# argmaxinc/WhisperKit

Hardware: NVIDIA H100
Metric: RTFx (audio-sec/s) whisper-large-v3 greedy (higher is better)
Workload: dtype bf16

## Files before the change

whisperkit_b200/csrc/decoder_ops.cu:

```cuda
#include <curand_kernel.h>
#include <math.h>

#include <stdlib.h>

#include "common.cuh"
#include <algorithm>
#include "kernels.h"

namespace wk {

static constexpr int kMaxCtx = 224;

__device__ __forceinline__ float block_sum(float v, float* scratch) {
    v = warp_sum(v);
    const int warp = threadIdx.x >> 5, lane = threadIdx.x & 31, nw = (blockDim.x + 31) >> 5;
    __syncthreads();
    if (lane == 0) scratch[warp] = v;
    __syncthreads();
    float r = (lane < nw) ? scratch[lane] : 0.f;
    r = warp_sum(r);
    return r;
}
__device__ __forceinline__ float block_max(float v, float* scratch) {
    v = warp_max(v);
    const int warp = threadIdx.x >> 5, lane = threadIdx.x & 31, nw = (blockDim.x + 31) >> 5;
    __syncthreads();
    if (lane == 0) scratch[warp] = v;
    __syncthreads();
    float r = (lane < nw) ? scratch[lane] : -INFINITY;
    r = warp_max(r);
    return r;
}

__global__ void decode_slots_init_kernel(DecodeState st, RowParams* __restrict__ rp_dev, const int32_t* __restrict__ slot_ids,
                                         const int32_t* __restrict__ prompts, const RowParams* __restrict__ rp_new, BeamState bs) {
    const int i = blockIdx.x, b = slot_ids[i];
    const RowParams R = rp_new[i];
    const int n_prompt = R.prompt_len;
    for (int t = threadIdx.x; t < kMaxCtx; t += blockDim.x) {
        st.tokens[b * kMaxCtx + t] = t < n_prompt ? prompts[i * kMaxCtx + t] : 0;
        st.logprobs[b * kMaxCtx + t] = 0.f;
    }
    if (threadIdx.x == 0) {
        rp_dev[b] = R;
        st.n_tokens[b] = n_prompt;
        st.next_token[b] = n_prompt > 0 ? prompts[i * kMaxCtx + n_prompt - 1] : 0;
        st.done[b] = 0;
        st.first_low[b] = 0;
        st.steps[b] = 0;
        st.input_ids[b] = 0;
        st.error[b] = 0;
        st.lang_token[b] = -1;
        st.lang_logprob[b] = 0.f;
        st.lang_state[b] = R.detect == 2 ? kLangLead : 0;
        st.no_speech[b] = __int_as_float(0x7fc00000);
        if (bs.beam > 1) {
            bs.sum_lp[b] = 0.f;
            if (b % bs.beam == 0) bs.n_fin[b / bs.beam] = 0;
        }
    }
}

wk_status decode_slots_init(DecodeState st, RowParams* rp_dev, const int32_t* slot_ids, const int32_t* prompts, const RowParams* rp_new,
                            int n, cudaStream_t stream, BeamState beam) {
    if (n < 1) return WK_OK;
    decode_slots_init_kernel<<<n, 64, 0, stream>>>(st, rp_dev, slot_ids, prompts, rp_new, beam);
    count_launch();
    cudaError_t e = cudaGetLastError();
    if (e != cudaSuccess) { set_error("decode_slots_init launch: %s", cudaGetErrorString(e)); return WK_ERR_CUDA; }
    return WK_OK;
}

template <typename T>
__global__ void __launch_bounds__(256)
decoder_embed_ln_kernel(const T* __restrict__ emb, const float* __restrict__ pos_emb, const float* __restrict__ gamma,
                        const float* __restrict__ beta, DecodeState st, int vocab, int ts_begin, float* __restrict__ x,
                        T* __restrict__ xn, int d, const int32_t* __restrict__ explicit_pos) {
    __shared__ float scratch[32];
    const int b = blockIdx.x, tid = threadIdx.x;
    pdl_launch_dependents();
    pdl_wait();
    int tok, pos;
    if (explicit_pos) {
        tok = st.input_ids[b];
        pos = explicit_pos[b];
    } else {
        if (st.done[b]) return;
        const int step = st.steps[b];
        const int prompt_len = st.rp[b].prompt_len;
        pos = step;
        tok = st.next_token[b];
        bool overwrite = false;
        const int lang_state = st.lang_state[b];
        if (lang_state == kLangLead) {
            tok = st.rp[b].lead_token;
        } else if (step < prompt_len) {
            const int cur = st.tokens[b * kMaxCtx + step];
            const bool is_ts = cur >= ts_begin, pred_ts = tok >= ts_begin;
            if (!(step == prompt_len - 1 && is_ts && pred_ts)) tok = cur;
            else overwrite = true;
        }
        __syncthreads();
        if (tid == 0) {
            if (overwrite) st.tokens[b * kMaxCtx + step] = tok;
            st.input_ids[b] = tok;
            if (lang_state == kLangLeadRan) st.lang_state[b] = 0;
        }
    }
    tok = min(max(tok, 0), vocab - 1);
    float v[8];
    float s = 0.f;
#pragma unroll
    for (int k = 0; k < 8; ++k) {
        const int i = tid + k * 256;
        v[k] = 0.f;
        if (i < d) {
            v[k] = T16<T>::to_f(emb[(long long)tok * d + i]) + pos_emb[(long long)pos * d + i];
            x[(long long)b * d + i] = v[k];
            s += v[k];
        }
    }
    const float mean = block_sum(s, scratch) / d;
    float q = 0.f;
#pragma unroll
    for (int k = 0; k < 8; ++k) {
        const int i = tid + k * 256;
        if (i < d) { const float a = v[k] - mean; q += a * a; }
    }
    const float rstd = rsqrtf(block_sum(q, scratch) / d + 1e-5f);
#pragma unroll
    for (int k = 0; k < 8; ++k) {
        const int i = tid + k * 256;
        if (i < d) xn[(long long)b * d + i] = T16<T>::from_f((v[k] - mean) * rstd * gamma[i] + beta[i]);
    }
}

wk_status decoder_embed_ln(const void* emb16, const float* pos, const float* gamma, const float* beta, DecodeState st, int vocab,
                           int ts_begin, float* x, void* xn, int B, int d, int dtype, const int32_t* explicit_pos, cudaStream_t stream) {
    if (d > 2048) { set_error("decoder_embed_ln: d_model %d > 2048", d); return WK_ERR_INVALID_ARGUMENT; }
    if (dtype == WK_DTYPE_F16)
        launch_k(decoder_embed_ln_kernel<__half>, dim3(B), dim3(256), 0, stream, 1, (const __half*)emb16, pos, gamma, beta, st, vocab, ts_begin, x, (__half*)xn, d, explicit_pos);
    else
        launch_k(decoder_embed_ln_kernel<__nv_bfloat16>, dim3(B), dim3(256), 0, stream, 1, (const __nv_bfloat16*)emb16, pos, gamma, beta, st, vocab, ts_begin, x, (__nv_bfloat16*)xn, d, explicit_pos);
    count_launch();
    cudaError_t e = cudaGetLastError();
    if (e != cudaSuccess) { set_error("decoder_embed_ln launch: %s", cudaGetErrorString(e)); return WK_ERR_CUDA; }
    return WK_OK;
}

static constexpr int kReduceThreads = 320;
static constexpr int kMaxSplits = 20;

template <typename T>
__global__ void __launch_bounds__(kReduceThreads)
decoder_reduce_resid_ln_kernel(const float* __restrict__ partial, int splits, int Bp, const float* __restrict__ bias,
                               const float* __restrict__ gamma, const float* __restrict__ beta, float* __restrict__ x,
                               T* __restrict__ xn, int d) {
    __shared__ float scratch[32];
    const int b = blockIdx.x, tid = threadIdx.x;
    const int d4 = d >> 2;
    pdl_launch_dependents();
    pdl_wait();
    float4 v[2];
    float s = 0.f;
#pragma unroll
    for (int k = 0; k < 2; ++k) {
        const int i4 = tid + k * kReduceThreads;
        v[k] = make_float4(0.f, 0.f, 0.f, 0.f);
        if (i4 < d4) {
            float4 p[kMaxSplits];
#pragma unroll
            for (int sp = 0; sp < kMaxSplits; ++sp)
                if (sp < splits) p[sp] = __ldcg(reinterpret_cast<const float4*>(partial + ((long long)sp * Bp + b) * d) + i4);
            float4 a = reinterpret_cast<const float4*>(x + (long long)b * d)[i4];
            if (bias) {
                const float4 bb = __ldg(reinterpret_cast<const float4*>(bias) + i4);
                a.x += bb.x; a.y += bb.y; a.z += bb.z; a.w += bb.w;
            }
#pragma unroll
            for (int sp = 0; sp < kMaxSplits; ++sp)
                if (sp < splits) { a.x += p[sp].x; a.y += p[sp].y; a.z += p[sp].z; a.w += p[sp].w; }
            v[k] = a;
            reinterpret_cast<float4*>(x + (long long)b * d)[i4] = a;
            s += a.x + a.y + a.z + a.w;
        }
    }
    const float mean = block_sum(s, scratch) / d;
    float q = 0.f;
#pragma unroll
    for (int k = 0; k < 2; ++k) {
        const int i4 = tid + k * kReduceThreads;
        if (i4 < d4) {
            const float a0 = v[k].x - mean, a1 = v[k].y - mean, a2 = v[k].z - mean, a3 = v[k].w - mean;
            q += a0 * a0 + a1 * a1 + a2 * a2 + a3 * a3;
        }
    }
    const float rstd = rsqrtf(block_sum(q, scratch) / d + 1e-5f);
#pragma unroll
    for (int k = 0; k < 2; ++k) {
        const int i4 = tid + k * kReduceThreads;
        if (i4 < d4) {
            const float4 g = __ldg(reinterpret_cast<const float4*>(gamma) + i4), bb = __ldg(reinterpret_cast<const float4*>(beta) + i4);
            uint2 pk;
            pk.x = T16<T>::pack2((v[k].x - mean) * rstd * g.x + bb.x, (v[k].y - mean) * rstd * g.y + bb.y);
            pk.y = T16<T>::pack2((v[k].z - mean) * rstd * g.z + bb.z, (v[k].w - mean) * rstd * g.w + bb.w);
            reinterpret_cast<uint2*>(xn + (long long)b * d)[i4] = pk;
        }
    }
}

wk_status decoder_reduce_resid_ln(const float* partial, int splits, int Bp, const float* bias, const float* gamma,
                                  const float* beta, float* x, void* xn, int B, int d, int dtype, cudaStream_t stream) {
    if (splits > kMaxSplits || d > 8 * kReduceThreads || (d & 3)) {
        set_error("decoder_reduce_resid_ln: unsupported splits %d / d %d", splits, d);
        return WK_ERR_INVALID_ARGUMENT;
    }
    if (dtype == WK_DTYPE_F16)
        launch_k(decoder_reduce_resid_ln_kernel<__half>, dim3(B), dim3(kReduceThreads), 0, stream, 32, partial, splits, Bp, bias, gamma, beta, x, (__half*)xn, d);
    else
        launch_k(decoder_reduce_resid_ln_kernel<__nv_bfloat16>, dim3(B), dim3(kReduceThreads), 0, stream, 32, partial, splits, Bp, bias, gamma, beta, x, (__nv_bfloat16*)xn, d);
    count_launch();
    cudaError_t e = cudaGetLastError();
    if (e != cudaSuccess) { set_error("decoder_reduce_resid_ln launch: %s", cudaGetErrorString(e)); return WK_ERR_CUDA; }
    return WK_OK;
}

template <typename T>
__global__ void __launch_bounds__(256)
decoder_reduce_bias_gelu_kernel(const float* __restrict__ partial, int splits, int Bp, const float* __restrict__ bias,
                                T* __restrict__ out, int B, int n) {
    pdl_launch_dependents();
    pdl_wait();
    const long long idx = ((long long)blockIdx.x * blockDim.x + threadIdx.x) * 4;
    if (idx >= (long long)B * n) return;
    const int b = (int)(idx / n), i = (int)(idx - (long long)b * n);
    float4 a = *reinterpret_cast<const float4*>(bias + i);
    float4 p[8];
#pragma unroll
    for (int sp = 0; sp < 8; ++sp)
        if (sp < splits) p[sp] = __ldcg(reinterpret_cast<const float4*>(partial + ((long long)sp * Bp + b) * n + i));
#pragma unroll
    for (int sp = 0; sp < 8; ++sp)
        if (sp < splits) { a.x += p[sp].x; a.y += p[sp].y; a.z += p[sp].z; a.w += p[sp].w; }
    for (int sp = 8; sp < splits; ++sp) {
        const float4 pp = __ldcg(reinterpret_cast<const float4*>(partial + ((long long)sp * Bp + b) * n + i));
        a.x += pp.x; a.y += pp.y; a.z += pp.z; a.w += pp.w;
    }
    uint2 pk;
    pk.x = T16<T>::pack2(gelu_erf(a.x), gelu_erf(a.y));
    pk.y = T16<T>::pack2(gelu_erf(a.z), gelu_erf(a.w));
    *reinterpret_cast<uint2*>(out + (long long)b * n + i) = pk;
}

wk_status decoder_reduce_bias_gelu(const float* partial, int splits, int Bp, const float* bias, void* out, int B, int n,
                                   int dtype, cudaStream_t stream) {
    const long long threads = (long long)B * n / 4;
    const unsigned grid = (unsigned)((threads + 255) / 256);
    if (dtype == WK_DTYPE_F16)
        launch_k(decoder_reduce_bias_gelu_kernel<__half>, dim3(grid), dim3(256), 0, stream, 32, partial, splits, Bp, bias, (__half*)out, B, n);
    else
        launch_k(decoder_reduce_bias_gelu_kernel<__nv_bfloat16>, dim3(grid), dim3(256), 0, stream, 32, partial, splits, Bp, bias, (__nv_bfloat16*)out, B, n);
    count_launch();
    cudaError_t e = cudaGetLastError();
    if (e != cudaSuccess) { set_error("decoder_reduce_bias_gelu launch: %s", cudaGetErrorString(e)); return WK_ERR_CUDA; }
    return WK_OK;
}

template <typename T, bool kAnc>
__global__ void __launch_bounds__(128)
decoder_self_attention_kernel(const float* __restrict__ partial, int splits, int Bp, const float* __restrict__ bq,
                              const float* __restrict__ bv, T* __restrict__ kcache, T* __restrict__ vcache,
                              const int32_t* __restrict__ pos_ptr, const int32_t* __restrict__ done,
                              T* __restrict__ out, int B, int H, int max_len, const int32_t* __restrict__ anc) {
    __shared__ float sq[64], skc[64], svc[64];
    __shared__ float sp[kMaxCtx];
    __shared__ float red[4][64];
    __shared__ float sstat[8];
    const int tid = threadIdx.x, warp = tid >> 5, lane = tid & 31;
    const int bh = blockIdx.x, b = bh / H, h = bh % H;
    pdl_launch_dependents();
    pdl_wait();
    if (done != nullptr && done[b]) return;
    const int dm = H * 64;
    const int pos = pos_ptr[b];
    const int32_t* arow = kAnc ? anc + (long long)b * max_len : nullptr;
    const long long own = (long long)bh * max_len;
    auto row_of = [&](int t) -> long long { return kAnc ? ((long long)arow[t] * H + h) * max_len + t : own + t; };
    if (warp == 0) {
        const int e = 2 * lane;
        float2 q = make_float2(bq[h * 64 + e], bq[h * 64 + e + 1]);
        float2 k = make_float2(0.f, 0.f);
        float2 v = make_float2(bv[h * 64 + e], bv[h * 64 + e + 1]);
        for (int s = 0; s < splits; ++s) {
            const float* pr = partial + ((long long)s * Bp + b) * (3LL * dm) + h * 64 + e;
            const float2 pq = *reinterpret_cast<const float2*>(pr);
            const float2 pk = *reinterpret_cast<const float2*>(pr + dm);
            const float2 pv = *reinterpret_cast<const float2*>(pr + 2 * dm);
            q.x += pq.x; q.y += pq.y; k.x += pk.x; k.y += pk.y; v.x += pv.x; v.y += pv.y;
        }
        const uint32_t k16 = T16<T>::pack2(k.x, k.y), v16 = T16<T>::pack2(v.x, v.y);
        *reinterpret_cast<uint32_t*>(kcache + (own + pos) * 64 + e) = k16;
        *reinterpret_cast<uint32_t*>(vcache + (own + pos) * 64 + e) = v16;
        const float2 kr = T16<T>::unpack2(k16), vr = T16<T>::unpack2(v16);
        sq[e] = q.x; sq[e + 1] = q.y;
        skc[e] = kr.x; skc[e + 1] = kr.y;
        svc[e] = vr.x; svc[e + 1] = vr.y;
        const float self = warp_sum(q.x * kr.x + q.y * kr.y);
        if (lane == 0) sp[pos] = self * 0.125f;
    }
    __syncthreads();
    const int sub = lane & 7, rsel = lane >> 3;
    float qv[8];
#pragma unroll
    for (int j = 0; j < 8; ++j) qv[j] = sq[sub * 8 + j];
    const T* kb = kcache + sub * 8;
#pragma unroll 4
    for (int t0 = warp * 4; t0 < pos; t0 += 16) {
        const int t = t0 + rsel;
        float acc = 0.f;
        if (t < pos) {
            const uint4 u = *reinterpret_cast<const uint4*>(kb + row_of(t) * 64);
            const float2 a0 = T16<T>::unpack2(u.x), a1 = T16<T>::unpack2(u.y), a2 = T16<T>::unpack2(u.z), a3 = T16<T>::unpack2(u.w);
            acc = qv[0] * a0.x + qv[1] * a0.y + qv[2] * a1.x + qv[3] * a1.y + qv[4] * a2.x + qv[5] * a2.y + qv[6] * a3.x + qv[7] * a3.y;
        }
        acc += __shfl_xor_sync(0xffffffffu, acc, 1);
        acc += __shfl_xor_sync(0xffffffffu, acc, 2);
        acc += __shfl_xor_sync(0xffffffffu, acc, 4);
        if (sub == 0 && t < pos) sp[t] = acc * 0.125f;
    }
    __syncthreads();
    float mx = -INFINITY;
    for (int t = tid; t <= pos; t += 128) mx = fmaxf(mx, sp[t]);
    mx = warp_max(mx);
    if (lane == 0) sstat[warp] = mx;
    __syncthreads();
    mx = fmaxf(fmaxf(sstat[0], sstat[1]), fmaxf(sstat[2], sstat[3]));
    float sm = 0.f;
    for (int t = tid; t <= pos; t += 128) {
        const float pr = __expf(sp[t] - mx);
        sp[t] = pr;
        sm += pr;
    }
    sm = warp_sum(sm);
    if (lane == 0) sstat[4 + warp] = sm;
    __syncthreads();
    const float inv = 1.f / (sstat[4] + sstat[5] + sstat[6] + sstat[7]);
    float o8[8];
#pragma unroll
    for (int j = 0; j < 8; ++j) o8[j] = 0.f;
    const T* vb = vcache + sub * 8;
#pragma unroll 4
    for (int t0 = warp * 4; t0 < pos; t0 += 16) {
        const int t = t0 + rsel;
        if (t < pos) {
            const float pr = sp[t];
            const uint4 u = *reinterpret_cast<const uint4*>(vb + row_of(t) * 64);
            const float2 a0 = T16<T>::unpack2(u.x), a1 = T16<T>::unpack2(u.y), a2 = T16<T>::unpack2(u.z), a3 = T16<T>::unpack2(u.w);
            o8[0] += pr * a0.x; o8[1] += pr * a0.y; o8[2] += pr * a1.x; o8[3] += pr * a1.y;
            o8[4] += pr * a2.x; o8[5] += pr * a2.y; o8[6] += pr * a3.x; o8[7] += pr * a3.y;
        }
    }
#pragma unroll
    for (int j = 0; j < 8; ++j) {
        o8[j] += __shfl_xor_sync(0xffffffffu, o8[j], 8);
        o8[j] += __shfl_xor_sync(0xffffffffu, o8[j], 16);
    }
    if (rsel == 0) {
#pragma unroll
        for (int j = 0; j < 8; ++j) red[warp][sub * 8 + j] = o8[j];
    }
    __syncthreads();
    if (tid < 64) {
        const float o = red[0][tid] + red[1][tid] + red[2][tid] + red[3][tid] + sp[pos] * svc[tid];
        out[(long long)b * dm + h * 64 + tid] = T16<T>::from_f(o * inv);
    }
}

wk_status decoder_self_attention(const float* partial, int splits, int Bp, const float* bq, const float* bv, void* kcache,
                                 void* vcache, const int32_t* pos, const int32_t* done, void* out, int B, int H,
                                 int max_len, int dtype, cudaStream_t stream, const int32_t* anc) {
    if (max_len > kMaxCtx) { set_error("decoder_self_attention: max_len %d > %d", max_len, kMaxCtx); return WK_ERR_INVALID_ARGUMENT; }
    const unsigned grid = (unsigned)(B * H);
    if (dtype == WK_DTYPE_F16) {
        if (anc) launch_k(decoder_self_attention_kernel<__half, true>, dim3(grid), dim3(128), 0, stream, 2, partial, splits, Bp, bq, bv, (__half*)kcache, (__half*)vcache, pos, done, (__half*)out, B, H, max_len, anc);
        else launch_k(decoder_self_attention_kernel<__half, false>, dim3(grid), dim3(128), 0, stream, 2, partial, splits, Bp, bq, bv, (__half*)kcache, (__half*)vcache, pos, done, (__half*)out, B, H, max_len, anc);
    } else {
        if (anc) launch_k(decoder_self_attention_kernel<__nv_bfloat16, true>, dim3(grid), dim3(128), 0, stream, 2, partial, splits, Bp, bq, bv, (__nv_bfloat16*)kcache, (__nv_bfloat16*)vcache, pos, done, (__nv_bfloat16*)out, B, H, max_len, anc);
        else launch_k(decoder_self_attention_kernel<__nv_bfloat16, false>, dim3(grid), dim3(128), 0, stream, 2, partial, splits, Bp, bq, bv, (__nv_bfloat16*)kcache, (__nv_bfloat16*)vcache, pos, done, (__nv_bfloat16*)out, B, H, max_len, anc);
    }
    count_launch();
    cudaError_t e = cudaGetLastError();
    if (e != cudaSuccess) { set_error("decoder_self_attention launch: %s", cudaGetErrorString(e)); return WK_ERR_CUDA; }
    return WK_OK;
}

template <bool FP8> struct CrossCfg {
    static constexpr int kRowBytes = FP8 ? 64 : 128;
    static constexpr int kRows = FP8 ? 250 : 125;
    static constexpr int kStageBytes = kRows * kRowBytes;
    static constexpr int kStages = FP8 ? 3 : 4;
    static constexpr int kLanesPerRow = kRowBytes / 16;
    static constexpr int kRowsPerWarp = 32 / kLanesPerRow;
    static constexpr int kDims = 64 / kLanesPerRow;
};
static constexpr int kCrossRows = CrossCfg<false>::kRows;
static constexpr int kCrossThreads = 160;

__device__ __forceinline__ void fp8x16_to_f32(const uint4 u, float (&x)[16]) {
    const uint32_t w[4] = {u.x, u.y, u.z, u.w};
#pragma unroll
    for (int k = 0; k < 4; ++k) {
        uint32_t lo, hi;
        fp8x4_to_half2(w[k], lo, hi);
        const float2 a = T16<__half>::unpack2(lo), b = T16<__half>::unpack2(hi);
        x[4 * k] = a.x; x[4 * k + 1] = a.y; x[4 * k + 2] = b.x; x[4 * k + 3] = b.y;
    }
}
template <typename T, bool FP8>
__device__ __forceinline__ float cross_row_dot(const uint8_t* piece, const float (&qv)[CrossCfg<FP8>::kDims]) {
    const uint4 u = *reinterpret_cast<const uint4*>(piece);
    if constexpr (FP8) {
        float x[16];
        fp8x16_to_f32(u, x);
        float acc = 0.f;
#pragma unroll
        for (int j = 0; j < 16; ++j) acc = fmaf(qv[j], x[j], acc);
        return acc;
    } else {
        const float2 a0 = T16<T>::unpack2(u.x), a1 = T16<T>::unpack2(u.y), a2 = T16<T>::unpack2(u.z), a3 = T16<T>::unpack2(u.w);
        return qv[0] * a0.x + qv[1] * a0.y + qv[2] * a1.x + qv[3] * a1.y + qv[4] * a2.x + qv[5] * a2.y + qv[6] * a3.x + qv[7] * a3.y;
    }
}
template <typename T, bool FP8>
__device__ __forceinline__ void cross_row_axpy(const uint8_t* piece, float p, float (&acc)[CrossCfg<FP8>::kDims]) {
    const uint4 u = *reinterpret_cast<const uint4*>(piece);
    if constexpr (FP8) {
        float x[16];
        fp8x16_to_f32(u, x);
#pragma unroll
        for (int j = 0; j < 16; ++j) acc[j] = fmaf(p, x[j], acc[j]);
    } else {
        const float2 a0 = T16<T>::unpack2(u.x), a1 = T16<T>::unpack2(u.y), a2 = T16<T>::unpack2(u.z), a3 = T16<T>::unpack2(u.w);
        acc[0] += p * a0.x; acc[1] += p * a0.y; acc[2] += p * a1.x; acc[3] += p * a1.y;
        acc[4] += p * a2.x; acc[5] += p * a2.y; acc[6] += p * a3.x; acc[7] += p * a3.y;
    }
}

template <typename T, bool FP8>
__global__ void __launch_bounds__(kCrossThreads)
decoder_cross_attention_kernel(const float* __restrict__ partial, int splits, int Bp, const float* __restrict__ bq,
                               const uint8_t* __restrict__ kcross, const uint8_t* __restrict__ vcross, const float* __restrict__ kscale,
                               const float* __restrict__ vscale, T* __restrict__ out, int B, int H, int Tlen, const int32_t* __restrict__ done,
                               float* __restrict__ align_scratch, uint32_t align_mask, int kv_div) {
    using C = CrossCfg<FP8>;
    extern __shared__ __align__(128) uint8_t smem[];
    const int Tp = (Tlen + 3) & ~3;
    uint8_t* ring = smem;
    float* scores = reinterpret_cast<float*>(smem + C::kStages * C::kStageBytes);
    float* ksc = scores + Tp;
    float* vsc = ksc + Tp;
    float* sq = FP8 ? vsc + Tp : scores + Tp;
    float* red = sq + 64;
    uint64_t* full_bar = reinterpret_cast<uint64_t*>(red + 4 * 64 + 32);
    uint64_t* empty_bar = full_bar + C::kStages;
    uint64_t* scale_bar = empty_bar + C::kStages;

    const int tid = threadIdx.x, warp = tid >> 5, lane = tid & 31;
    const int beam_j = blockIdx.x % kv_div, wh = blockIdx.x / kv_div;
    const int win = wh / H, h = wh % H, b = win * kv_div + beam_j;
    const int kvh = win * H + h;
    const int dm = H * 64;
    const int chunks = Tlen / C::kRows;
    pdl_launch_dependents();
    const int ended = done != nullptr ? done[b] : 0;
    if (tid == 0) {
        for (int i = 0; i < C::kStages; ++i) { mbar_init(&full_bar[i], 1); mbar_init(&empty_bar[i], 4); }
        if constexpr (FP8) mbar_init(scale_bar, 1);
        fence_barrier_init();
    }
    __syncthreads();
    if (ended) { pdl_wait(); return; }

    if (warp == 4) {
        if (lane == 0) {
            if constexpr (FP8) {
                mbar_expect_tx(scale_bar, 2u * Tlen * 4);
                bulk_load_1d(ksc, kscale + (long long)kvh * Tlen, Tlen * 4, scale_bar);
                bulk_load_1d(vsc, vscale + (long long)kvh * Tlen, Tlen * 4, scale_bar);
            }
            const uint8_t* kb = kcross + (long long)kvh * Tlen * C::kRowBytes;
            const uint8_t* vb = vcross + (long long)kvh * Tlen * C::kRowBytes;
            for (int c = 0; c < 2 * chunks; ++c) {
                const int stage = c % C::kStages;
                const uint32_t ph = (c / C::kStages) & 1;
                mbar_wait(&empty_bar[stage], ph ^ 1);
                mbar_expect_tx(&full_bar[stage], C::kStageBytes);
                const uint8_t* src = c < chunks ? kb + (long long)c * C::kStageBytes : vb + (long long)(c - chunks) * C::kStageBytes;
                bulk_load_1d(ring + stage * C::kStageBytes, src, C::kStageBytes, &full_bar[stage]);
            }
        }
        return;
    }
    pdl_wait();
    if (tid < 64) {
        float q = bq[h * 64 + tid];
        for (int s = 0; s < splits; ++s) q += partial[((long long)s * Bp + b) * dm + h * 64 + tid];
        sq[tid] = q * 0.125f;
    }
    asm volatile("bar.sync 1, 128;" ::: "memory");
    const int sub = lane % C::kLanesPerRow;
    const int rsel = lane / C::kLanesPerRow;
    float qv[C::kDims];
#pragma unroll
    for (int j = 0; j < C::kDims; ++j) qv[j] = sq[sub * C::kDims + j];
    if constexpr (FP8) mbar_wait(scale_bar, 0);

// ... 597 lines not shown
```

whisperkit_b200/csrc/gemm_wgmma.cu:

```cuda
#include <stdarg.h>
#include <stdio.h>
#include <stdlib.h>

#include <algorithm>

#include "common.cuh"
#include "kernels.h"
#include "wgmma.cuh"

namespace wk {

static constexpr int kBlockM = 128;
static constexpr int kBlockK = 64;
static constexpr int kStageA = kBlockM * kBlockK * 2;
static constexpr int kGemmThreads = 384;
static constexpr int kMaxStages = 10;
static constexpr int kSmemMax = 227 * 1024;

struct GemmKParams {
    int tiles_per_batch, n_batches, tiles_n, splits, work;
    int kb_per_tap, kb_per_split, taps;
    int tap_row_shift[3];
    int tap_col_off[3];
    int a_is_3d;
    int m_rows_per_batch, n, bn;
    int stage_b_bytes, stages, store_bytes;
    int mode, gelu;
    void* out;
    long long ld_out, out_rows_per_batch, partial_cols;
    const float* bias;
    const float* pos;
    long long ld_pos;
    int heads_T, heads_B, heads_H, heads_dmodel;
    float* out_scale;
    int a_static;
};

enum GemmEpi { kEpiPartialT = 0, kEpiFp8Heads = 1, kEpiStore16 = 2, kEpiStore32 = 3 };
static int gemm_epi(int mode) {
    switch (mode) {
        case GEMM_OUT_PARTIAL_T: return kEpiPartialT;
        case GEMM_OUT_FP8_HEADS: return kEpiFp8Heads;
        case GEMM_OUT_T16: case GEMM_OUT_T16_HEADS: return kEpiStore16;
        default: return kEpiStore32;
    }
}

static constexpr int kStoreBox = 64 * 128;
static constexpr int kStoreBytes = 2  * 2  * kStoreBox;

__device__ __forceinline__ uint32_t swz128(int row, int chunk) { return (uint32_t)(row * 128 + ((chunk ^ (row & 7)) << 4)); }

__device__ __forceinline__ void store_box_begin(int wg_tid, int cw) {
    fence_proxy_async();
    if (wg_tid == 0) bulk_wait_read_all();
    warpgroup_bar(1 + cw);
}

template <typename T, int BN>
__device__ __forceinline__ void gemm_epilogue_store16(const GemmKParams& p, const CUtensorMap* tmO, const float (&acc)[BN / 2],
                                                      uint8_t* stage, int& sbuf, int wg_tid, int cw, int batch, int row0, int col_base) {
    const int lane = wg_tid & 31;
    const int q = lane & 3;
    const int mrow = 16 * (wg_tid >> 5) + 8 * ((lane >> 3) & 1) + (lane & 7);
    const int mj = lane >> 4;
    const bool heads = p.mode == GEMM_OUT_T16_HEADS;
    int hb = 0, ht0 = 0;
    bool straddle = false;
    if (heads) {
        hb = row0 / p.heads_T;
        ht0 = row0 - hb * p.heads_T;
        straddle = ht0 + 64 > p.heads_T && (hb + 1) * p.heads_T < p.m_rows_per_batch;
    }
#pragma unroll
    for (int c = 0; c < BN / 64; ++c) {
        const int col0 = col_base + 64 * c;
        if (col0 >= p.n) break;
        uint8_t* buf = stage + sbuf * kStoreBox;
        const uint32_t sb = smem_u32(buf);
#pragma unroll
        for (int jp = 0; jp < 4; ++jp) {
            uint32_t r[4];
#pragma unroll
            for (int h = 0; h < 2; ++h) {
                const int j = 8 * c + 2 * jp + h;
                const int col = col_base + 8 * j + 2 * q;
                float v0 = acc[4 * j], v1 = acc[4 * j + 1], v2 = acc[4 * j + 2], v3 = acc[4 * j + 3];
                if (p.bias && col < p.n) {
                    const float2 bb = __ldg(reinterpret_cast<const float2*>(p.bias + col));
                    v0 += bb.x; v1 += bb.y; v2 += bb.x; v3 += bb.y;
                }
                if (p.gelu) {
                    const float2 g0 = gelu_erf2(make_float2(v0, v1)), g1 = gelu_erf2(make_float2(v2, v3));
                    v0 = g0.x; v1 = g0.y; v2 = g1.x; v3 = g1.y;
                }
                r[2 * h] = T16<T>::pack2(v0, v1);
                r[2 * h + 1] = T16<T>::pack2(v2, v3);
            }
            stmatrix_x4(sb + swz128(mrow, 2 * jp + mj), r[0], r[1], r[2], r[3]);
        }
        store_box_begin(wg_tid, cw);
        int blk = 0;
        if (heads) {
            const int which = col0 / p.heads_dmodel;
            blk = (which * p.heads_B + hb) * p.heads_H + ((col0 - which * p.heads_dmodel) >> 6);
        }
        if (wg_tid == 0) {
            if (heads) tma_store_3d(tmO, buf, 0, ht0, blk);
            else tma_store_3d(tmO, buf, col0, row0, batch);
            bulk_commit();
        }
        if (straddle) {
            const int s = p.heads_T - ht0;
            uint8_t* dst = reinterpret_cast<uint8_t*>(p.out) + (long long)(blk + p.heads_H) * p.heads_T * 128;
            for (int i = wg_tid; i < (64 - s) * 8; i += 128) {
                const int r = s + (i >> 3), ch = i & 7;
                *reinterpret_cast<uint4*>(dst + (long long)(r - s) * 128 + ch * 16) = *reinterpret_cast<const uint4*>(buf + swz128(r, ch));
            }
        }
        sbuf ^= 1;
    }
}

template <int BN>
__device__ __forceinline__ void gemm_epilogue_store32(const GemmKParams& p, const CUtensorMap* tmO, const float (&acc)[BN / 2],
                                                      uint8_t* stage, uint64_t* rbar, int& sbuf, uint32_t& rphase, int wg_tid, int cw,
                                                      int batch, int row0, int col_base) {
    const int lane = wg_tid & 31;
    const int q = lane & 3;
    const int r_top = 16 * (wg_tid >> 5) + (lane >> 2);
    const bool add = p.mode == GEMM_OUT_F32_ADD, pos = p.mode == GEMM_OUT_F32_GELU_POS;
#pragma unroll
    for (int c = 0; c < BN / 32; ++c) {
        const int col0 = col_base + 32 * c;
        if (col0 >= p.n) break;
        uint8_t* buf = stage + sbuf * kStoreBox;
        if (add) {
            if (wg_tid == 0 && c >= 1 && c + 1 < BN / 32 && col0 + 32 < p.n) {
                bulk_wait_read_all();
                mbar_expect_tx(&rbar[sbuf ^ 1], kStoreBox);
                tma_load_3d(stage + (sbuf ^ 1) * kStoreBox, tmO, &rbar[sbuf ^ 1], col0 + 32, row0, batch);
            }
            mbar_wait(&rbar[sbuf], (rphase >> sbuf) & 1u);
            rphase ^= 1u << sbuf;
        }
#pragma unroll
        for (int jj = 0; jj < 4; ++jj) {
            const int j = 4 * c + jj;
            const int col = col_base + 8 * j + 2 * q;
            float v[4] = {acc[4 * j], acc[4 * j + 1], acc[4 * j + 2], acc[4 * j + 3]};
            if (p.bias && col < p.n) {
                const float2 bb = __ldg(reinterpret_cast<const float2*>(p.bias + col));
                v[0] += bb.x; v[1] += bb.y; v[2] += bb.x; v[3] += bb.y;
            }
            if (p.gelu) {
                const float2 g0 = gelu_erf2(make_float2(v[0], v[1])), g1 = gelu_erf2(make_float2(v[2], v[3]));
                v[0] = g0.x; v[1] = g0.y; v[2] = g1.x; v[3] = g1.y;
            }
#pragma unroll
            for (int half = 0; half < 2; ++half) {
                const int r = r_top + 8 * half;
                float2* s = reinterpret_cast<float2*>(buf + swz128(r, 2 * jj + (q >> 1)) + (q & 1) * 8);
                float2 o = make_float2(v[2 * half], v[2 * half + 1]);
                if (add) {
                    const float2 x = *s;
                    o = make_float2(x.x + o.x, x.y + o.y);
                } else if (pos) {
                    const int row_in_batch = row0 + r;
                    if (row_in_batch < p.m_rows_per_batch && col < p.n) {
                        const float2 pp = __ldg(reinterpret_cast<const float2*>(p.pos + (long long)row_in_batch * p.ld_pos + col));
                        o = make_float2(o.x + pp.x, o.y + pp.y);
                    }
                }
                *s = o;
            }
        }
        store_box_begin(wg_tid, cw);
        if (wg_tid == 0) {
            tma_store_3d(tmO, buf, col0, row0, batch);
            bulk_commit();
        }
        sbuf ^= 1;
    }
}

template <int BN>
__device__ __forceinline__ void gemm_epilogue_fp8_heads(const GemmKParams& p, int batch, int tile_row0, int r_lo, int c_lo, int col_base,
                                                        const float (&acc)[BN / 2]) {
    static_assert(BN % 64 == 0, "FP8 heads epilogue needs head-aligned N tiles");
#pragma unroll
    for (int half = 0; half < 2; ++half) {
        const int row_in_batch = tile_row0 + r_lo + 8 * half;
        const long long grow = (long long)batch * p.out_rows_per_batch + row_in_batch;
        const int b = (int)(grow / p.heads_T);
        const int tt = (int)(grow - (long long)b * p.heads_T);
#pragma unroll
        for (int hh = 0; hh < BN / 64; ++hh) {
            const int col0 = col_base + hh * 64;
            const bool col_ok = col0 < p.n;
            float v[16];
            float amax = 0.f;
#pragma unroll
            for (int jj = 0; jj < 8; ++jj) {
                const int j = hh * 8 + jj;
                float v0 = acc[4 * j + 2 * half], v1 = acc[4 * j + 2 * half + 1];
                if (p.bias && col_ok) {
                    const float2 bb = __ldg(reinterpret_cast<const float2*>(p.bias + col0 + 8 * jj + c_lo));
                    v0 += bb.x; v1 += bb.y;
                }
                v[2 * jj] = v0; v[2 * jj + 1] = v1;
                amax = fmaxf(amax, fmaxf(fabsf(v0), fabsf(v1)));
            }
            amax = fmaxf(amax, __shfl_xor_sync(0xffffffffu, amax, 1));
            amax = fmaxf(amax, __shfl_xor_sync(0xffffffffu, amax, 2));
            if (!col_ok || row_in_batch >= p.m_rows_per_batch) continue;
            const int which = col0 / p.heads_dmodel;
            const int h = (col0 - which * p.heads_dmodel) >> 6;
            const long long row = (((long long)which * p.heads_B + b) * p.heads_H + h) * p.heads_T + tt;
            const float s = fp8_row_scale(amax);
            uint8_t* o = reinterpret_cast<uint8_t*>(p.out) + row * 64 + c_lo;
#pragma unroll
            for (int jj = 0; jj < 8; ++jj)
                *reinterpret_cast<uint16_t*>(o + 8 * jj) = (uint16_t)(fp8_encode(v[2 * jj], s) | (fp8_encode(v[2 * jj + 1], s) << 8));
            if (c_lo == 0) p.out_scale[row] = s;
        }
    }
}

template <typename T, int BN, int EPI>
__global__ void __launch_bounds__(kGemmThreads, 1)
gemm_wgmma_kernel(const __grid_constant__ CUtensorMap tmA, const __grid_constant__ CUtensorMap tmB, const __grid_constant__ CUtensorMap tmO,
                  const GemmKParams p) {
    constexpr bool kStore = EPI == kEpiStore16 || EPI == kEpiStore32;
    extern __shared__ __align__(1024) uint8_t smem_raw[];
    uint8_t* smem = reinterpret_cast<uint8_t*>((reinterpret_cast<uintptr_t>(smem_raw) + 1023) & ~uintptr_t(1023));
    const int stage_bytes = kStageA + p.stage_b_bytes;
    uint8_t* store_stage = smem + (size_t)p.stages * stage_bytes;
    uint64_t* full_bar = reinterpret_cast<uint64_t*>(store_stage + p.store_bytes);
    uint64_t* empty_bar = full_bar + kMaxStages;
    uint64_t* res_bar = empty_bar + kMaxStages;

    const int warp = threadIdx.x >> 5;
    const int lane = threadIdx.x & 31;
    pdl_launch_dependents();

    if (warp == 0 && lane == 0) {
        tma_prefetch_desc(&tmA);
        tma_prefetch_desc(&tmB);
        if (kStore) tma_prefetch_desc(&tmO);
        for (int i = 0; i < p.stages; ++i) {
            mbar_init(&full_bar[i], 1);
            mbar_init(&empty_bar[i], 8);
        }
        for (int i = 0; i < 4; ++i) mbar_init(&res_bar[i], 1);
        fence_barrier_init();
    }
    __syncthreads();
    const bool early_a = p.a_static != 0;
    if (!(early_a && warp == 0)) pdl_wait();

    if (warp < 4) {
        asm volatile("setmaxnreg.dec.sync.aligned.u32 40;");
        if (warp != 0) return;
        int stage = 0;
        uint32_t phase = 0;
        bool need_wait = early_a;
        auto issue = [&](int kb, int st, int row0, int batch, int n_tile, bool do_a, bool do_b) {
            const int tap = kb / p.kb_per_tap;
            const int kk = kb - tap * p.kb_per_tap;
            uint8_t* sa = smem + (size_t)st * stage_bytes;
            uint8_t* sb = sa + kStageA;
            if (do_a) {
                mbar_expect_tx_elect(&full_bar[st], (uint32_t)stage_bytes);
                const int ac0 = p.tap_col_off[tap] + kk * kBlockK;
                const int ar = row0 + p.tap_row_shift[tap];
                if (p.a_is_3d) tma_load_3d_elect(sa, &tmA, &full_bar[st], ac0, ar, batch);
                else tma_load_2d_elect(sa, &tmA, &full_bar[st], ac0, ar);
            }
            if (do_b) tma_load_2d_elect(sb, &tmB, &full_bar[st], kb * kBlockK, n_tile * BN);
        };
        for (int w = blockIdx.x; w < p.work; w += gridDim.x) {
            const int split = w % p.splits;
            const int t = w / p.splits;
            const int n_tile = t % p.tiles_n;
            const int m_tile = t / p.tiles_n;
            const int batch = m_tile / p.tiles_per_batch;
            const int row0 = (m_tile % p.tiles_per_batch) * kBlockM;
            const int kb0 = split * p.kb_per_split;
            int kb = kb0;
            if (need_wait) {
                const int n_pre = p.kb_per_split < p.stages ? p.kb_per_split : p.stages;
                for (int i = 0; i < n_pre; ++i) issue(kb0 + i, i, row0, batch, n_tile, true, false);
                pdl_wait();
                for (int i = 0; i < n_pre; ++i) issue(kb0 + i, i, row0, batch, n_tile, false, true);
                kb = kb0 + n_pre;
                if (n_pre == p.stages) { stage = 0; phase ^= 1; } else stage = n_pre;
                need_wait = false;
            }
            for (; kb < kb0 + p.kb_per_split; ++kb) {
                mbar_wait(&empty_bar[stage], phase ^ 1);
                __syncwarp();
                issue(kb, stage, row0, batch, n_tile, true, true);
                if (++stage == p.stages) { stage = 0; phase ^= 1; }
            }
        }
        if (need_wait) pdl_wait();
        return;
    }

    asm volatile("setmaxnreg.inc.sync.aligned.u32 232;");
    const int cw = (warp >> 2) - 1;
    const int wg_tid = threadIdx.x & 127;
    const int r_lo = cw * 64 + (warp & 3) * 16 + (lane >> 2);
    const int c_lo = 2 * (lane & 3);
    uint8_t* my_stage = store_stage + cw * 2 * kStoreBox;
    uint64_t* my_res_bar = res_bar + 2 * cw;
    int sbuf = 0;
    uint32_t rphase = 0;
    int stage = 0;
    uint32_t phase = 0;
    float acc[BN / 2];
    for (int w = blockIdx.x; w < p.work; w += gridDim.x) {
        const int split = w % p.splits;
        const int t = w / p.splits;
        const int n_tile = t % p.tiles_n;
        const int m_tile = t / p.tiles_n;
        const int batch = m_tile / p.tiles_per_batch;
        const int tile_row0 = (m_tile % p.tiles_per_batch) * kBlockM;
        const int col_base = n_tile * BN;
        const int wg_row0 = tile_row0 + 64 * cw;
        const bool wg_rows = wg_row0 < p.m_rows_per_batch;

        int prev = -1;
        for (int kb = 0; kb < p.kb_per_split; ++kb) {
            mbar_wait(&full_bar[stage], phase);
            const uint32_t sa = smem_u32(smem + (size_t)stage * stage_bytes);
            const uint64_t adesc = wgmma_desc_sw128(sa + cw * 64 * 128);
            const uint64_t bdesc = wgmma_desc_sw128(sa + kStageA);
            wgmma_fence();
#pragma unroll
            for (int k = 0; k < kBlockK / 16; ++k)
                Wgmma<T, BN>::ss(acc, adesc + (uint64_t)(2 * k), bdesc + (uint64_t)(2 * k), (kb > 0 || k > 0) ? 1u : 0u);
            wgmma_commit();
            if (EPI == kEpiStore32 && kb == 0 && p.mode == GEMM_OUT_F32_ADD && wg_tid == 0 && wg_rows) {
                bulk_wait_read_all();
                for (int c = 0; c < 2 && c < BN / 32 && col_base + 32 * c < p.n; ++c) {
                    const int b = sbuf ^ c;
                    mbar_expect_tx(&my_res_bar[b], kStoreBox);
                    tma_load_3d(my_stage + b * kStoreBox, &tmO, &my_res_bar[b], col_base + 32 * c, wg_row0, batch);
                }
            }
            wgmma_wait<1>();
            if (prev >= 0) {
                __syncwarp();
                if (lane == 0) mbar_arrive(&empty_bar[prev]);
            }
            prev = stage;
            if (++stage == p.stages) { stage = 0; phase ^= 1; }
        }
        wgmma_wait<0>();
        __syncwarp();
        if (lane == 0) mbar_arrive(&empty_bar[prev]);

        if constexpr (EPI == kEpiFp8Heads) {
            gemm_epilogue_fp8_heads<BN>(p, batch, tile_row0, r_lo, c_lo, col_base, acc);
        } else if constexpr (EPI == kEpiStore16) {
            if (wg_rows) gemm_epilogue_store16<T, BN>(p, &tmO, acc, my_stage, sbuf, wg_tid, cw, batch, wg_row0, col_base);
        } else if constexpr (EPI == kEpiStore32) {
            if (wg_rows) gemm_epilogue_store32<BN>(p, &tmO, acc, my_stage, my_res_bar, sbuf, rphase, wg_tid, cw, batch, wg_row0, col_base);
        } else {
            float* o = reinterpret_cast<float*>(p.out);
#pragma unroll
            for (int half = 0; half < 2; ++half) {
                const int row_in_batch = tile_row0 + r_lo + 8 * half;
                if (row_in_batch >= p.m_rows_per_batch) continue;
                const long long grow = (long long)batch * p.out_rows_per_batch + row_in_batch;
#pragma unroll
                for (int j = 0; j < BN / 8; ++j) {
                    const int col = col_base + 8 * j + c_lo;
                    if (col < p.partial_cols) o[((long long)split * p.partial_cols + col) * p.ld_out + grow] = acc[4 * j + 2 * half];
                    if (col + 1 < p.partial_cols) o[((long long)split * p.partial_cols + col + 1) * p.ld_out + grow] = acc[4 * j + 2 * half + 1];
                }
            }
        }
    }
    if (kStore && wg_tid == 0) bulk_wait_all();
}

typedef CUresult (*PFN_encodeTiled)(CUtensorMap*, CUtensorMapDataType, cuuint32_t, void*, const cuuint64_t*, const cuuint64_t*,
                                    const cuuint32_t*, const cuuint32_t*, CUtensorMapInterleave, CUtensorMapSwizzle,
                                    CUtensorMapL2promotion, CUtensorMapFloatOOBfill);

static PFN_encodeTiled get_encode_fn() {
    static PFN_encodeTiled fn = nullptr;
    if (!fn) {
        void* p = nullptr;
        cudaDriverEntryPointQueryResult q;
        if (cudaGetDriverEntryPoint("cuTensorMapEncodeTiled", &p, cudaEnableDefault, &q) == cudaSuccess &&
            q == cudaDriverEntryPointSuccess)
            fn = reinterpret_cast<PFN_encodeTiled>(p);
    }
    return fn;
}

static wk_status make_tmap(CUtensorMap* tm, const void* base, int dtype, int ndim, const uint64_t* dims,
                           const uint64_t* strides_bytes, const uint32_t* box) {
    PFN_encodeTiled enc = get_encode_fn();
    if (!enc) {
        set_error("cuTensorMapEncodeTiled entry point unavailable (no CUDA driver?)");
        return WK_ERR_CUDA;
    }
    cuuint64_t gdim[3];
    cuuint64_t gstr[2];
    cuuint32_t bx[3];
    cuuint32_t es[3] = {1, 1, 1};
    for (int i = 0; i < ndim; ++i) { gdim[i] = dims[i]; bx[i] = box[i]; }
    for (int i = 0; i < ndim - 1; ++i) gstr[i] = strides_bytes[i];
    const CUtensorMapDataType ty = dtype == WK_DTYPE_F32 ? CU_TENSOR_MAP_DATA_TYPE_FLOAT32
                                   : dtype == WK_DTYPE_F16 ? CU_TENSOR_MAP_DATA_TYPE_FLOAT16 : CU_TENSOR_MAP_DATA_TYPE_BFLOAT16;
    CUresult r = enc(tm, ty,
                     (cuuint32_t)ndim, const_cast<void*>(base), gdim, gstr, bx, es, CU_TENSOR_MAP_INTERLEAVE_NONE,
                     CU_TENSOR_MAP_SWIZZLE_128B, CU_TENSOR_MAP_L2_PROMOTION_L2_256B, CU_TENSOR_MAP_FLOAT_OOB_FILL_NONE);
    if (r != CUDA_SUCCESS) {
        set_error("cuTensorMapEncodeTiled failed: %d (ndim %d dims %llu %llu stride %llu box %u %u)", (int)r, ndim,
                  (unsigned long long)dims[0], (unsigned long long)dims[1], (unsigned long long)strides_bytes[0], box[0],
                  box[1]);
        return WK_ERR_CUDA;
    }
    return WK_OK;
}

wk_status make_tmap_2d(void* tm, const void* base, int dtype, uint64_t cols, uint64_t rows, uint64_t ld_elems, uint32_t box_cols, uint32_t box_rows) {
    uint64_t dims[2] = {cols, rows};
    uint64_t str[1] = {ld_elems * 2};
    uint32_t box[2] = {box_cols, box_rows};
    return make_tmap(reinterpret_cast<CUtensorMap*>(tm), base, dtype, 2, dims, str, box);
}

int wgmma_tile_n(int bn) {
    int t = 16;
    while (t < bn) t <<= 1;
    return t;
}

template <typename T, int BN, int EPI>
static cudaError_t launch_gemm(const CUtensorMap& tmA, const CUtensorMap& tmB, const CUtensorMap& tmO, const GemmKParams& p, int grid,
                               size_t smem, int pdl, cudaStream_t stream) {
    static bool attr_set = false;
    if (!attr_set) {
        const cudaError_t e = cudaFuncSetAttribute(gemm_wgmma_kernel<T, BN, EPI>, cudaFuncAttributeMaxDynamicSharedMemorySize, kSmemMax);
        if (e != cudaSuccess) return e;
        attr_set = true;
    }
    return launch_k(gemm_wgmma_kernel<T, BN, EPI>, dim3(grid), dim3(kGemmThreads), smem, stream, pdl, tmA, tmB, tmO, p);
}

template <typename T, int EPI>
static cudaError_t launch_gemm_store(const CUtensorMap& tmA, const CUtensorMap& tmB, const CUtensorMap& tmO, const GemmKParams& p, int grid,
                                     size_t smem, int pdl, cudaStream_t stream) {
    switch (p.bn) {
        case 64: return launch_gemm<T, 64, EPI>(tmA, tmB, tmO, p, grid, smem, pdl, stream);
        case 128: return launch_gemm<T, 128, EPI>(tmA, tmB, tmO, p, grid, smem, pdl, stream);
        default: return launch_gemm<T, 256, EPI>(tmA, tmB, tmO, p, grid, smem, pdl, stream);
    }
}

template <typename T>
static cudaError_t launch_gemm_n(const CUtensorMap& tmA, const CUtensorMap& tmB, const CUtensorMap& tmO, const GemmKParams& p, int grid,
                                 size_t smem, int pdl, cudaStream_t stream) {
    switch (gemm_epi(p.mode)) {
        case kEpiFp8Heads: return launch_gemm<T, 256, kEpiFp8Heads>(tmA, tmB, tmO, p, grid, smem, pdl, stream);
        case kEpiStore16: return launch_gemm_store<T, kEpiStore16>(tmA, tmB, tmO, p, grid, smem, pdl, stream);
        case kEpiStore32: return launch_gemm_store<T, kEpiStore32>(tmA, tmB, tmO, p, grid, smem, pdl, stream);
        default: break;
    }
    switch (p.bn) {
        case 16: return launch_gemm<T, 16, kEpiPartialT>(tmA, tmB, tmO, p, grid, smem, pdl, stream);
        case 32: return launch_gemm<T, 32, kEpiPartialT>(tmA, tmB, tmO, p, grid, smem, pdl, stream);
        case 64: return launch_gemm<T, 64, kEpiPartialT>(tmA, tmB, tmO, p, grid, smem, pdl, stream);
        case 128: return launch_gemm<T, 128, kEpiPartialT>(tmA, tmB, tmO, p, grid, smem, pdl, stream);
        default: return launch_gemm<T, 256, kEpiPartialT>(tmA, tmB, tmO, p, grid, smem, pdl, stream);
    }
}

wk_status gemm_wgmma(const GemmDesc& d, int num_sms, cudaStream_t stream) {
    if (d.k % kBlockK != 0 || d.bn % 16 != 0 || d.bn < 16 || d.bn > 256 || d.taps < 1 || d.taps > 3) {
        set_error("gemm_wgmma: unsupported shape k=%d bn=%d taps=%d", d.k, d.bn, d.taps);
        return WK_ERR_INVALID_ARGUMENT;
    }
    if (d.mode != GEMM_OUT_PARTIAL_T && (d.n % 32 != 0 || d.splits != 1)) {
        set_error("gemm_wgmma: n=%d must be a multiple of 32 and splits 1 for mode %d", d.n, d.mode);
        return WK_ERR_INVALID_ARGUMENT;
    }
    GemmKParams p;
    memset(&p, 0, sizeof(p));
    p.kb_per_tap = d.k / kBlockK;
    const int total_kb = p.kb_per_tap * d.taps;
    p.splits = d.splits < 1 ? 1 : d.splits;
    if (total_kb % p.splits != 0) {
        set_error("gemm_wgmma: splits %d does not divide %d k-blocks", p.splits, total_kb);
        return WK_ERR_INVALID_ARGUMENT;
    }
    p.kb_per_split = total_kb / p.splits;
    p.taps = d.taps;
    for (int i = 0; i < 3; ++i) { p.tap_row_shift[i] = d.tap_row_shift[i]; p.tap_col_off[i] = d.tap_col_off[i]; }
    p.a_is_3d = d.a_3d ? 1 : 0;
    p.n_batches = d.a_3d ? d.a_batches : 1;
    p.m_rows_per_batch = d.m_rows_per_batch;
    p.tiles_per_batch = (d.m_rows_per_batch + kBlockM - 1) / kBlockM;
    p.n = d.n;
    p.bn = wgmma_tile_n(d.bn);
    const int epi = gemm_epi(d.mode);
    const bool tma_store = epi == kEpiStore16 || epi == kEpiStore32;
    if (tma_store && p.bn < 64) p.bn = 64;
    p.tiles_n = (d.n + p.bn - 1) / p.bn;
    p.work = p.tiles_per_batch * p.n_batches * p.tiles_n * p.splits;
    p.stage_b_bytes = p.bn * kBlockK * 2;
    if (p.stage_b_bytes % 1024 != 0) p.stage_b_bytes = (p.stage_b_bytes + 1023) / 1024 * 1024;
    const int stage_bytes = kStageA + p.stage_b_bytes;
    p.store_bytes = tma_store ? kStoreBytes : 0;
    const int smem_budget = kSmemMax - 1024  - 256  - p.store_bytes;
    int stages = smem_budget / stage_bytes;
    if (stages > kMaxStages) stages = kMaxStages;
    if (stages > total_kb / p.splits + 2) stages = total_kb / p.splits + 2;
    if (stages < 2) stages = 2;
    if (d.max_stages > 0 && stages > d.max_stages) stages = d.max_stages;
    p.stages = stages;
    p.a_static = d.a_static;
    p.mode = d.mode;
    p.gelu = d.gelu;
    p.out = d.out;
    p.ld_out = d.ld_out;
    p.out_rows_per_batch = d.out_rows_per_batch;
    p.partial_cols = d.partial_cols;
    p.bias = d.bias;
    p.pos = d.pos;
    p.ld_pos = d.ld_pos;
    p.heads_T = d.heads_T; p.heads_B = d.heads_B; p.heads_H = d.heads_H; p.heads_dmodel = d.heads_dmodel;
    p.out_scale = d.out_scale;
    if (d.mode == GEMM_OUT_FP8_HEADS && (p.bn != 256 || d.n % 64 != 0 || d.heads_dmodel % 64 != 0 || !d.out_scale)) {
        set_error("gemm_wgmma: the FP8 heads epilogue needs 256-column tiles and head-aligned columns (bn %d n %d d %d)", p.bn, d.n, d.heads_dmodel);
        return WK_ERR_INVALID_ARGUMENT;
    }
    if (d.mode == GEMM_OUT_T16_HEADS &&
        (p.n_batches != 1 || d.n % 64 != 0 || d.heads_dmodel % 64 != 0 || d.n % d.heads_dmodel != 0 || d.m_rows_per_batch % d.heads_T != 0)) {
        set_error("gemm_wgmma: the 16-bit heads epilogue needs head-aligned columns and whole windows (n %d d %d rows %d T %d)", d.n,
                  d.heads_dmodel, d.m_rows_per_batch, d.heads_T);
        return WK_ERR_INVALID_ARGUMENT;
    }

    CUtensorMap tmA, tmB, tmO;
    memset(&tmO, 0, sizeof(tmO));
    wk_status st;
    if (p.a_is_3d) {
        uint64_t dims[3] = {(uint64_t)d.a_cols, (uint64_t)d.a_rows, (uint64_t)d.a_batches};
        uint64_t str[2] = {(uint64_t)d.a_ld * 2, (uint64_t)d.a_batch_stride * 2};
        uint32_t box[3] = {kBlockK, kBlockM, 1};
        st = make_tmap(&tmA, d.a, d.in_dtype, 3, dims, str, box);
    } else {
        uint64_t dims[2] = {(uint64_t)d.a_cols, (uint64_t)d.a_rows};
        uint64_t str[1] = {(uint64_t)d.a_ld * 2};
        uint32_t box[2] = {kBlockK, kBlockM};
        st = make_tmap(&tmA, d.a, d.in_dtype, 2, dims, str, box);
    }
    if (st != WK_OK) return st;
    {
        uint64_t dims[2] = {(uint64_t)d.k * d.taps, (uint64_t)d.b_rows};
        uint64_t str[1] = {(uint64_t)d.b_ld * 2};
        uint32_t box[2] = {kBlockK, (uint32_t)p.bn};
        st = make_tmap(&tmB, d.b, d.in_dtype, 2, dims, str, box);
        if (st != WK_OK) return st;
    }
    if (d.mode == GEMM_OUT_T16_HEADS) {
        uint64_t dims[3] = {64, (uint64_t)d.heads_T, (uint64_t)(d.n / d.heads_dmodel) * d.heads_B * d.heads_H};
        uint64_t str[2] = {128, (uint64_t)d.heads_T * 128};
        uint32_t box[3] = {64, 64, 1};
        st = make_tmap(&tmO, d.out, d.in_dtype, 3, dims, str, box);
    } else if (tma_store) {
        const int out_dtype = epi == kEpiStore16 ? d.in_dtype : WK_DTYPE_F32;
        const uint64_t es = epi == kEpiStore16 ? 2 : 4;
        uint64_t dims[3] = {(uint64_t)d.n, (uint64_t)d.m_rows_per_batch, (uint64_t)p.n_batches};
        uint64_t str[2] = {(uint64_t)d.ld_out * es, (uint64_t)d.out_rows_per_batch * d.ld_out * es};
        uint32_t box[3] = {(uint32_t)(128 / es), 64, 1};
        st = make_tmap(&tmO, d.out, out_dtype, 3, dims, str, box);
    }
    if (st != WK_OK) return st;
    const size_t smem_bytes = (size_t)stages * stage_bytes + p.store_bytes + 1024 + 256;
    int grid = p.work < num_sms ? p.work : num_sms;
    if (grid < 1) return WK_OK;
    const int pdl = d.pdl != 0 ? 16 : 0;
    cudaError_t e = d.in_dtype == WK_DTYPE_F16 ? launch_gemm_n<__half>(tmA, tmB, tmO, p, grid, smem_bytes, pdl, stream)
                                               : launch_gemm_n<__nv_bfloat16>(tmA, tmB, tmO, p, grid, smem_bytes, pdl, stream);
    count_launch();
    if (e == cudaSuccess) e = cudaGetLastError();
    if (e != cudaSuccess) {
        set_error("gemm_wgmma launch: %s", cudaGetErrorString(e));
        return WK_ERR_CUDA;
    }
    return WK_OK;
}

}
```

Measured before the change: 907.0.

## Tune decoder GEMM register split and single-pass reduce-LN kernel occupancy

Rewrites the split-K reduce + residual + LayerNorm kernel so each thread handles one float4 instead of looping over two, issues the x/bias loads alongside the partial-sum loads, and requests two blocks per SM. This lowers the supported d to 4*320=1280, which still covers whisper-large-v3. For the partial-output (split-K decoder) GEMM variant it drops the setmaxnreg producer/consumer register rebalancing and the min-blocks launch bound. It also pads dynamic shared memory to at least 116 KB, apparently to force one CTA per SM. The aim is to cut latency in the small-batch decoder path, at the risk of register spills in the GEMM consumer warps now that they no longer get the raised register budget.

```diff
diff --git a/whisperkit_b200/csrc/decoder_ops.cu b/whisperkit_b200/csrc/decoder_ops.cu
--- a/whisperkit_b200/csrc/decoder_ops.cu
+++ b/whisperkit_b200/csrc/decoder_ops.cu
@@ -152,66 +152,51 @@
 static constexpr int kMaxSplits = 20;
 
 template <typename T>
-__global__ void __launch_bounds__(kReduceThreads)
+__global__ void __launch_bounds__(kReduceThreads, 2)
 decoder_reduce_resid_ln_kernel(const float* __restrict__ partial, int splits, int Bp, const float* __restrict__ bias,
                                const float* __restrict__ gamma, const float* __restrict__ beta, float* __restrict__ x,
                                T* __restrict__ xn, int d) {
     __shared__ float scratch[32];
-    const int b = blockIdx.x, tid = threadIdx.x;
-    const int d4 = d >> 2;
+    const int b = blockIdx.x, i4 = threadIdx.x;
+    const bool live = i4 < (d >> 2);
     pdl_launch_dependents();
     pdl_wait();
-    float4 v[2];
+    float4 v = make_float4(0.f, 0.f, 0.f, 0.f);
     float s = 0.f;
-#pragma unroll
-    for (int k = 0; k < 2; ++k) {
-        const int i4 = tid + k * kReduceThreads;
-        v[k] = make_float4(0.f, 0.f, 0.f, 0.f);
-        if (i4 < d4) {
-            float4 p[kMaxSplits];
-#pragma unroll
-            for (int sp = 0; sp < kMaxSplits; ++sp)
-                if (sp < splits) p[sp] = __ldcg(reinterpret_cast<const float4*>(partial + ((long long)sp * Bp + b) * d) + i4);
-            float4 a = reinterpret_cast<const float4*>(x + (long long)b * d)[i4];
-            if (bias) {
-                const float4 bb = __ldg(reinterpret_cast<const float4*>(bias) + i4);
-                a.x += bb.x; a.y += bb.y; a.z += bb.z; a.w += bb.w;
-            }
-#pragma unroll
-            for (int sp = 0; sp < kMaxSplits; ++sp)
-                if (sp < splits) { a.x += p[sp].x; a.y += p[sp].y; a.z += p[sp].z; a.w += p[sp].w; }
-            v[k] = a;
-            reinterpret_cast<float4*>(x + (long long)b * d)[i4] = a;
-            s += a.x + a.y + a.z + a.w;
-        }
+    if (live) {
+        v = reinterpret_cast<const float4*>(x + (long long)b * d)[i4];
+        const float4 bb = bias ? __ldg(reinterpret_cast<const float4*>(bias) + i4) : make_float4(0.f, 0.f, 0.f, 0.f);
+        float4 p[kMaxSplits];
+#pragma unroll
+        for (int sp = 0; sp < kMaxSplits; ++sp)
+            if (sp < splits) p[sp] = __ldcg(reinterpret_cast<const float4*>(partial + ((long long)sp * Bp + b) * d) + i4);
+        __threadfence_block();
+        if (bias) { v.x += bb.x; v.y += bb.y; v.z += bb.z; v.w += bb.w; }
+#pragma unroll
+        for (int sp = 0; sp < kMaxSplits; ++sp)
+            if (sp < splits) { v.x += p[sp].x; v.y += p[sp].y; v.z += p[sp].z; v.w += p[sp].w; }
+        reinterpret_cast<float4*>(x + (long long)b * d)[i4] = v;
+        s = v.x + v.y + v.z + v.w;
     }
     const float mean = block_sum(s, scratch) / d;
     float q = 0.f;
-#pragma unroll
-    for (int k = 0; k < 2; ++k) {
-        const int i4 = tid + k * kReduceThreads;
-        if (i4 < d4) {
-            const float a0 = v[k].x - mean, a1 = v[k].y - mean, a2 = v[k].z - mean, a3 = v[k].w - mean;
-            q += a0 * a0 + a1 * a1 + a2 * a2 + a3 * a3;
-        }
+    if (live) {
+        const float a0 = v.x - mean, a1 = v.y - mean, a2 = v.z - mean, a3 = v.w - mean;
+        q = a0 * a0 + a1 * a1 + a2 * a2 + a3 * a3;
     }
     const float rstd = rsqrtf(block_sum(q, scratch) / d + 1e-5f);
-#pragma unroll
-    for (int k = 0; k < 2; ++k) {
-        const int i4 = tid + k * kReduceThreads;
-        if (i4 < d4) {
-            const float4 g = __ldg(reinterpret_cast<const float4*>(gamma) + i4), bb = __ldg(reinterpret_cast<const float4*>(beta) + i4);
-            uint2 pk;
-            pk.x = T16<T>::pack2((v[k].x - mean) * rstd * g.x + bb.x, (v[k].y - mean) * rstd * g.y + bb.y);
-            pk.y = T16<T>::pack2((v[k].z - mean) * rstd * g.z + bb.z, (v[k].w - mean) * rstd * g.w + bb.w);
-            reinterpret_cast<uint2*>(xn + (long long)b * d)[i4] = pk;
-        }
+    if (live) {
+        const float4 g = __ldg(reinterpret_cast<const float4*>(gamma) + i4), bb = __ldg(reinterpret_cast<const float4*>(beta) + i4);
+        uint2 pk;
+        pk.x = T16<T>::pack2((v.x - mean) * rstd * g.x + bb.x, (v.y - mean) * rstd * g.y + bb.y);
+        pk.y = T16<T>::pack2((v.z - mean) * rstd * g.z + bb.z, (v.w - mean) * rstd * g.w + bb.w);
+        reinterpret_cast<uint2*>(xn + (long long)b * d)[i4] = pk;
     }
 }
 
 wk_status decoder_reduce_resid_ln(const float* partial, int splits, int Bp, const float* bias, const float* gamma,
                                   const float* beta, float* x, void* xn, int B, int d, int dtype, cudaStream_t stream) {
-    if (splits > kMaxSplits || d > 8 * kReduceThreads || (d & 3)) {
+    if (splits > kMaxSplits || d > 4 * kReduceThreads || (d & 3)) {
         set_error("decoder_reduce_resid_ln: unsupported splits %d / d %d", splits, d);
         return WK_ERR_INVALID_ARGUMENT;
     }
diff --git a/whisperkit_b200/csrc/gemm_wgmma.cu b/whisperkit_b200/csrc/gemm_wgmma.cu
--- a/whisperkit_b200/csrc/gemm_wgmma.cu
+++ b/whisperkit_b200/csrc/gemm_wgmma.cu
@@ -16,6 +16,7 @@
 static constexpr int kGemmThreads = 384;
 static constexpr int kMaxStages = 10;
 static constexpr int kSmemMax = 227 * 1024;
+static constexpr int kDecoderGemmMinSmem = 116 * 1024;
 
 struct GemmKParams {
     int tiles_per_batch, n_batches, tiles_n, splits, work;
@@ -227,8 +228,14 @@
     }
 }
 
+template <int EPI>
+struct GemmRegs {
+    static constexpr bool kSplit = EPI != kEpiPartialT;
+    static constexpr int kMinBlocks = kSplit ? 1 : 0;
+};
+
 template <typename T, int BN, int EPI>
-__global__ void __launch_bounds__(kGemmThreads, 1)
+__global__ void __launch_bounds__(kGemmThreads, GemmRegs<EPI>::kMinBlocks)
 gemm_wgmma_kernel(const __grid_constant__ CUtensorMap tmA, const __grid_constant__ CUtensorMap tmB, const __grid_constant__ CUtensorMap tmO,
                   const GemmKParams p) {
     constexpr bool kStore = EPI == kEpiStore16 || EPI == kEpiStore32;
@@ -260,7 +267,7 @@
     if (!(early_a && warp == 0)) pdl_wait();
 
     if (warp < 4) {
-        asm volatile("setmaxnreg.dec.sync.aligned.u32 40;");
+        if constexpr (GemmRegs<EPI>::kSplit) asm volatile("setmaxnreg.dec.sync.aligned.u32 40;");
         if (warp != 0) return;
         int stage = 0;
         uint32_t phase = 0;
@@ -308,7 +315,7 @@
         return;
     }
 
-    asm volatile("setmaxnreg.inc.sync.aligned.u32 232;");
+    if constexpr (GemmRegs<EPI>::kSplit) asm volatile("setmaxnreg.inc.sync.aligned.u32 232;");
     const int cw = (warp >> 2) - 1;
     const int wg_tid = threadIdx.x & 127;
     const int r_lo = cw * 64 + (warp & 3) * 16 + (lane >> 2);
@@ -585,7 +592,8 @@
         st = make_tmap(&tmO, d.out, out_dtype, 3, dims, str, box);
     }
     if (st != WK_OK) return st;
-    const size_t smem_bytes = (size_t)stages * stage_bytes + p.store_bytes + 1024 + 256;
+    size_t smem_bytes = (size_t)stages * stage_bytes + p.store_bytes + 1024 + 256;
+    if (epi == kEpiPartialT && smem_bytes < kDecoderGemmMinSmem) smem_bytes = kDecoderGemmMinSmem;
     int grid = p.work < num_sms ? p.work : num_sms;
     if (grid < 1) return WK_OK;
     const int pdl = d.pdl != 0 ? 16 : 0;
```

Result: faster. 926.7, median of 6 (+2.2%).
